# samuelskirvin/EIGENSOLVER

Measured on AMD Instinct MI355X. Metric: det(M) evals/sec + roots/sec, 4096x4096 (k,omega) grid, higher is better.
Workload: dtype f64

## Files before the change

### eigensolver_amd/csrc/es_shoot.hip

```cpp
#include <vector>
#include <cstdio>
#include <cstdlib>
#include <cmath>
#include <type_traits>

#include "es_shoot_shared.hpp"

namespace {
using namespace es_shoot_shared;

struct GridOpts {
  int skip;
  const int* cols;
  int part;
  int main_span;
};

constexpr long ES_TILE_GRID_X = 1L << 22;
__device__ __forceinline__ long es_tile_index() { return (long)blockIdx.y * ES_TILE_GRID_X + blockIdx.x; }
inline dim3 es_tile_grid(long tiles) {
  return tiles <= ES_TILE_GRID_X ? dim3((unsigned)tiles) : dim3((unsigned)ES_TILE_GRID_X, (unsigned)((tiles + ES_TILE_GRID_X - 1) / ES_TILE_GRID_X));
}

template <int FAM, int PTS, int MAXT, bool TRACK, int WPE = 0>
// ... 16 lines not shown
  constexpr int MAXT = 256;
#include "es_shoot_grid_body.hpp"
}

__device__ __forceinline__ bool column_dead(const ShootDev& P, double W) {
  const double m = 4.0 * 2.220446049250313e-16 * fabs(W);
  bool c = false;
  for (int t = 0; t < P.n_bands; ++t) {
    const bool some = (W - m > P.band[t][0]) && (W + m < P.band[t][3]);
    const bool notall = (W + m <= P.band[t][1]) || (W - m >= P.band[t][2]);
    c = c || (some && notall);
  }
  return c;
}

__global__ __launch_bounds__(1024) void column_classify_kernel(ShootDev P, const double* __restrict__ Wv, int nw,
                                                               int* __restrict__ cols, uint8_t* __restrict__ dead) {
  __shared__ int wave_cnt[16];
  __shared__ int base;
  const int tid = threadIdx.x, lane = tid & 63, wid = tid >> 6;
  if (tid == 0) base = 0;
  __syncthreads();
  for (int j0 = 0; j0 < nw; j0 += 1024) {
    const int j = j0 + tid;
    const bool in = j < nw;
    const bool dd = in && column_dead(P, Wv[j]);
    if (in) dead[j] = dd ? 1 : 0;
    const bool live = in && !dd;
    const uint64_t m = __ballot(live);
    if (lane == 0) wave_cnt[wid] = __popcll(m);
    __syncthreads();
    int off = base;
    for (int v = 0; v < wid; ++v) off += wave_cnt[v];
    const uint64_t lower = (lane == 0) ? 0ull : (~0ull >> (64 - lane));
    if (live) cols[1 + off + __popcll(m & lower)] = j;
    __syncthreads();
    if (tid == 0) { int t = 0; for (int v = 0; v < 16; ++v) t += wave_cnt[v]; base += t; }
    __syncthreads();
  }
  if (tid == 0) cols[0] = base;
}

__global__ __launch_bounds__(256) void fill_dead_columns_kernel(ShootDev P, const double* __restrict__ kv, int nk,
                                                                const double* __restrict__ wv, int nw,
                                                                const uint8_t* __restrict__ dead,
                                                                double* __restrict__ Dout, double* __restrict__ relout,
                                                                uint8_t* __restrict__ stout) {
  const long cells = (long)nk * nw;
  for (long c = (long)blockIdx.x * blockDim.x + threadIdx.x; c < cells; c += (long)gridDim.x * blockDim.x) {
    const long row = c / nw;
    const int j = (int)(c - row * nw);
    if (!dead[j]) continue;
    const double k = kv[row];
    const double w = k * wv[j];
    const double k2 = k * k;
    const double Oe = (P.family == FAM_CYL0 || P.family == FAM_CYLT) ? w : (w - k * P.U_e);
    const double Oe2 = Oe * Oe;
    const double m_e = ((k2 * P.vAe2 - Oe2) * (k2 * P.ce2 - Oe2)) / (P.Se * (k2 * P.cTe2 - Oe2));
    const double cst = (P.family == FAM_CYL0 || P.family == FAM_CYLT)
                           ? -1.0 / (P.rho_e * (k2 * P.vAe2 - w * w))
                           : P.rho_e * P.Se * (k2 * P.cTe2 - Oe2) / (Oe * (k2 * P.ce2 - Oe2));
    uint8_t st = ES_PT_CONTINUUM;
    if (m_e < 0.0) st = ES_PT_LEAKY;
    else if (!(m_e > 0.0) || !isfinite(m_e) || !isfinite(cst)) st = ES_PT_NONFINITE;
    Dout[c] = NAN;
    if (relout) relout[c] = NAN;
    stout[c] = st;
  }
}

template <int FAM>
__global__ __launch_bounds__(256) void shoot_points_kernel(ShootDev P, const double* __restrict__ kv,
                                                           const double* __restrict__ wv, const int* __restrict__ d_n,
                                                           int n_max, double* __restrict__ Dout,
                                                           double* __restrict__ relout, uint8_t* __restrict__ stout) {
  ES_POINT_LDS(FAM);
  const int n = es_count(d_n, n_max);
  if ((long)blockIdx.x * 256 >= (long)n) return;
  const int i = blockIdx.x * blockDim.x + threadIdx.x;
  const bool in = i < n;
  const double k = in ? kv[i] : 1.0;
  const double w = in ? wv[i] : 1.0;
  double D, rel; uint8_t st;
  shoot_point<FAM>(P, k, w, w, D, rel, st, es_point_lds);
  if (in) {
    Dout[i] = D;
    stout[i] = st;
    if (relout) relout[i] = rel;
  }
}

__global__ __launch_bounds__(256) void bracket_flag_kernel(const double* __restrict__ D,
                                                           const uint8_t* __restrict__ st, int nw, long cells,
                                                           uint64_t* __restrict__ masks,
                                                           int* __restrict__ block_counts) {
  __shared__ int wave_cnt[4];
  const long c = (long)blockIdx.x * 256 + threadIdx.x;
  const int lane = threadIdx.x & 63;
  double d0 = 0.0; int ok0 = 0;
  if (c < cells) { d0 = D[c]; ok0 = (st[c] == ES_PT_OK); }
  double d1 = __shfl_down(d0, 1);
  int ok1 = __shfl_down(ok0, 1);
  if (lane == 63) {
    if (c + 1 < cells) { d1 = D[c + 1]; ok1 = (st[c + 1] == ES_PT_OK); } else { d1 = 0.0; ok1 = 0; }
  }
  bool flag = false;
  if (c < cells) {
    const long row = c / nw;
    const int j = (int)(c - row * nw);
    flag = (j < nw - 1) && ok0 && ok1 && (d0 * d1 < 0.0);
  }
  const uint64_t m = __ballot(flag);
  if (lane == 0) {
    masks[c >> 6] = m;
    wave_cnt[threadIdx.x >> 6] = __popcll(m);
  }
  __syncthreads();
  if (threadIdx.x == 0) block_counts[blockIdx.x] = wave_cnt[0] + wave_cnt[1] + wave_cnt[2] + wave_cnt[3];
}

__global__ __launch_bounds__(256) void bracket_emit_kernel(const double* __restrict__ kv,
                                                           const double* __restrict__ wv, int nw, int w_mode,
                                                           long cells, const double* __restrict__ D,
                                                           const uint64_t* __restrict__ masks,
                                                           const int* __restrict__ block_off, es_root_table tab,
                                                           double* __restrict__ d_lo_sign, double* __restrict__ d_hi_sign) {
  const long c = (long)blockIdx.x * 256 + threadIdx.x;
  if (c >= cells) return;
  const uint64_t m = masks[c >> 6];
  if (!((m >> (c & 63)) & 1ull)) return;
  const int pos = es_cell_rank(masks, block_off, c);
  if (pos >= tab.capacity) return;
  const long row = c / nw;
  const int j = (int)(c - row * nw);
  const double k = kv[row];
  tab.d_k[pos] = k;
  tab.d_row[pos] = (int32_t)row;
  tab.d_w_lo[pos] = pick_w(wv, w_mode, k, (int)row, nw, j);
  tab.d_w_hi[pos] = pick_w(wv, w_mode, k, (int)row, nw, j + 1);
  d_lo_sign[pos] = D[c];
  d_hi_sign[pos] = D[c + 1];
}

constexpr int kRefineSections = 17;
constexpr int kSharedMin = 0;

constexpr int REFINE_WAVES = 4;

template <int FAM, int LANES, int CHR = 0, bool SECTIONS_ONLY = false, bool ONE = false,
          int WPE = ((FAM == FAM_CYLT || !ONE) ? 2 : 3)>
__global__ __launch_bounds__(64 * REFINE_WAVES) __attribute__((amdgpu_waves_per_eu(WPE, WPE)))
void refine_kernel(ShootDev P, es_root_table tab, double* d_lo, double* d_hi, const int* __restrict__ d_n, int n_max,
                   int n_rounds, int n_polish, double tol_percent) {
  const int n = es_count(d_n, n_max);
  if ((int)(blockIdx.x * REFINE_WAVES * (64 / LANES)) >= n) return;
  constexpr int GROUPS = 64 / LANES;
  constexpr int WTBL = GROUPS * (2 * (CHR > 0 ? CHR : 1) + 1) * FamTraits<FAM>::NE;
  __shared__ double es_point_lds[CHR > 0 ? REFINE_WAVES * WTBL : FamTraits<FAM>::NB * (2 * es_shoot_shared::CH + 1)];
  const int lane = threadIdx.x & 63;
  const int g = lane / LANES, j = lane % LANES;
  const int i = (blockIdx.x * REFINE_WAVES + ((int)threadIdx.x >> 6)) * GROUPS + g;
  const bool in = i < n;
  const double k = in ? tab.d_k[i] : 1.0;
  double lo = in ? tab.d_w_lo[i] : 1.0;
  double hi = in ? tab.d_w_hi[i] : 2.0;
  double flo = in ? d_lo[i] : 1.0;
  double fhi = in ? d_hi[i] : -1.0;
  const double frac = (double)(j + 1) / (double)(LANES + 1);
  double D = 0.0, rel = 0.0; uint8_t st = 0;
  double root = lo;
  const int n_final = (n_polish > 0) ? n_polish : (n_polish == 0 ? 1 : 0);
  const int n_it = ONE ? 1 : n_rounds + n_final;
  for (int it = 0; it < n_it; ++it) {
    const bool section = ONE ? true : it < n_rounds;
    double x;
    if (section) {
      x = lo + (hi - lo) * frac;
    } else if (n_polish > 0) {
      x = lo - flo * (hi - lo) / (fhi - flo);
      if (!(x > lo && x < hi)) x = (x == x) ? ((fabs(flo) <= fabs(fhi)) ? lo : hi) : lo + (hi - lo) * 0.5;
    } else {
      x = lo + (hi - lo) * 0.5;
    }
    if (CHR > 0) shoot_point_wavegroup<FAM, (CHR > 0 ? CHR : 1), GROUPS>(P, k, x, D, rel, st, es_point_lds + ((int)threadIdx.x >> 6) * WTBL);
    else if (SECTIONS_ONLY) shoot_point<FAM, false>(P, k, x, x, D, rel, st, es_point_lds);
    else shoot_point<FAM>(P, k, x, x, D, rel, st, es_point_lds);
    if (section) {
      const bool diff = (D * flo < 0.0);
      const unsigned long long bal = __ballot(diff);
      const unsigned long long bits = (LANES == 64) ? bal : ((bal >> (LANES * g)) & ((1ull << (LANES & 63)) - 1ull));
      const int first = bits ? (__ffsll((long long)bits) - 1) : LANES;
      const int src_hi = g * LANES + (first < LANES ? first : LANES - 1);
      const int src_lo = g * LANES + (first > 0 ? first - 1 : 0);
      const double x_hi = __shfl(x, src_hi), d_hi_new = __shfl(D, src_hi);
      const double x_lo = __shfl(x, src_lo), d_lo_new = __shfl(D, src_lo);
      if (first < LANES) { hi = x_hi; fhi = d_hi_new; }
      if (first > 0) { lo = x_lo; flo = (d_lo_new == d_lo_new) ? d_lo_new : flo; }
    } else {
      root = x;
      if (n_polish > 0) {
        if (D * flo < 0.0) { hi = x; fhi = D; } else if (D == D) { lo = x; flo = D; }
      }
    }
  }
  if (in && j == 0) {
    tab.d_w_lo[i] = lo;
    tab.d_w_hi[i] = hi;
    if (n_polish < 0) {
      d_lo[i] = flo;
      d_hi[i] = fhi;
    } else {
      tab.d_w[i] = root;
      tab.d_resid[i] = rel;
      tab.d_flag[i] = (st == ES_PT_OK && rel < tol_percent) ? 1 : 0;
    }
  }
}

template <int FAM, bool ONE = false, int WPE = ((FAM == FAM_CYLT || !ONE) ? 2 : 3)>
__global__ __launch_bounds__(64 * REFINE_WAVES) __attribute__((amdgpu_waves_per_eu(WPE, WPE)))
void refine_polish_kernel(ShootDev P, es_root_table tab, double* d_lo, double* d_hi, const int* __restrict__ d_n,
                          int n_max, int n_polish, double tol_percent) {
  ES_POINT_LDS(FAM);
  const int n = es_count(d_n, n_max);
  if ((int)(blockIdx.x * (64 * REFINE_WAVES)) >= n) return;
  const int i = blockIdx.x * (64 * REFINE_WAVES) + (int)threadIdx.x;
  const bool in = i < n;
  const double k = in ? tab.d_k[i] : 1.0;
  double lo = in ? tab.d_w_lo[i] : 1.0;
  double hi = in ? tab.d_w_hi[i] : 2.0;
  double flo = in ? d_lo[i] : 1.0;
  double fhi = in ? d_hi[i] : -1.0;
  double D = 0.0, rel = 0.0; uint8_t st = 0;
  double root = lo;
  const int n_it = ONE ? 1 : n_polish;
  for (int it = 0; it < n_it; ++it) {
    double x = lo - flo * (hi - lo) / (fhi - flo);
    if (!(x > lo && x < hi)) x = (x == x) ? ((fabs(flo) <= fabs(fhi)) ? lo : hi) : lo + (hi - lo) * 0.5;
    shoot_point<FAM>(P, k, x, x, D, rel, st, es_point_lds);
    root = x;
    if (D * flo < 0.0) { hi = x; fhi = D; } else if (D == D) { lo = x; flo = D; }
  }
  if (in) {
    tab.d_w_lo[i] = lo;
    tab.d_w_hi[i] = hi;
    if (ONE && n_polish == 0) {
      d_lo[i] = flo;
      d_hi[i] = fhi;
    } else {
      tab.d_w[i] = root;
      tab.d_resid[i] = rel;
      tab.d_flag[i] = (st == ES_PT_OK && rel < tol_percent) ? 1 : 0;
    }
  }
}

constexpr int kHybridSections = 1;
constexpr int kHybridSteps = 8;
constexpr double kHybridEps = 1e-12;

struct HybridState {
  double* lo; double* hi; double* flo; double* fhi; double* xprev;
  int* info;
};
constexpr int HYB_ACTIVE = 0, HYB_KEPT = 1, HYB_FAILED = 2;

template <int FAM, int WPE = (FAM == FAM_CYL0 ? 3 : 2)>
__global__ __launch_bounds__(64 * REFINE_WAVES) __attribute__((amdgpu_waves_per_eu(WPE, WPE)))
void refine_superlinear_kernel(ShootDev P, es_root_table tab, const double* d_lo, const double* d_hi, HybridState S,
                               const int* __restrict__ d_n, int n_max, int step, double tol_percent,
                               unsigned long long* stats) {
  ES_POINT_LDS(FAM);
  const int n = es_count(d_n, n_max);
  if ((int)(blockIdx.x * (64 * REFINE_WAVES)) >= n) return;
  const int i = blockIdx.x * (64 * REFINE_WAVES) + (int)threadIdx.x;
  const bool in = i < n;
  const bool first = step == 0;
  const int info = (in && !first) ? S.info[i] : 0;
  const bool active = in && ((info >> 2) == HYB_ACTIVE);
  if (!__syncthreads_or(active ? 1 : 0)) return;
  const double k = in ? tab.d_k[i] : 1.0;
  double lo, hi, flo, fhi, xprev;
  if (first) {
    lo = in ? tab.d_w_lo[i] : 1.0;
    hi = in ? tab.d_w_hi[i] : 2.0;
    flo = in ? d_lo[i] : 1.0;
    fhi = in ? d_hi[i] : -1.0;
    xprev = NAN;
  } else {
    lo = active ? S.lo[i] : 1.0;
    hi = active ? S.hi[i] : 2.0;
    flo = active ? S.flo[i] : 1.0;
    fhi = active ? S.fhi[i] : -1.0;
    xprev = active ? S.xprev[i] : NAN;
  }
  int side = info & 3, status = info >> 2;
  double D = 0.0, rel = 0.0; uint8_t st = 0;
  double x = lo - flo * (hi - lo) / (fhi - flo);
  if (!(x > lo && x < hi)) x = lo + (hi - lo) * 0.5;
  shoot_point<FAM>(P, k, x, x, D, rel, st, es_point_lds);
  if (active) {
    if (D == D) {
      if (D * flo < 0.0) { hi = x; fhi = D; if (side == 1) flo *= 0.5; side = 1; }
      else { lo = x; flo = D; if (side == 2) fhi *= 0.5; side = 2; }
      const double ax = fabs(x);
      if (D == 0.0 || fabs(x - xprev) <= kHybridEps * ax || (hi - lo) <= kHybridEps * ax)
        status = (st == ES_PT_OK && rel < tol_percent) ? HYB_KEPT : HYB_FAILED;
    } else {
      status = HYB_FAILED;
    }
    if (status == HYB_KEPT) {
      tab.d_w_lo[i] = lo;
      tab.d_w_hi[i] = hi;
      tab.d_w[i] = x;
      tab.d_resid[i] = rel;
      tab.d_flag[i] = 1;
    } else if (status == HYB_ACTIVE) {
      S.lo[i] = lo; S.hi[i] = hi; S.flo[i] = flo; S.fhi[i] = fhi; S.xprev[i] = x;
    }
    S.info[i] = side | (status << 2);
  }
  const int n_eval = __popcll(__ballot(active)), n_kept = __popcll(__ballot(active && status == HYB_KEPT));
  if ((threadIdx.x & 63) == 0) {
    if (first && n_eval) atomicAdd(stats + 0, (unsigned long long)n_eval);
    if (n_kept) atomicAdd(stats + 1, (unsigned long long)n_kept);
    if (n_eval) atomicAdd(stats + 3, (unsigned long long)n_eval);
  }
}

__global__ __launch_bounds__(256) void hybrid_flag_kernel(const int* __restrict__ info, const int* __restrict__ d_n,
                                                          int n_max, uint64_t* __restrict__ masks,
                                                          int* __restrict__ block_counts, unsigned long long* stats) {
  __shared__ int wave_cnt[4];
  const int n = es_count(d_n, n_max);
  const int i = blockIdx.x * 256 + (int)threadIdx.x;
  const bool flag = i < n && (info[i] >> 2) != HYB_KEPT;
  const uint64_t m = __ballot(flag);
  if ((threadIdx.x & 63) == 0) {
    masks[i >> 6] = m;
    wave_cnt[threadIdx.x >> 6] = __popcll(m);
  }
  __syncthreads();
  if (threadIdx.x == 0) {
    const int c = wave_cnt[0] + wave_cnt[1] + wave_cnt[2] + wave_cnt[3];
    block_counts[blockIdx.x] = c;
    if (c) atomicAdd(stats + 2, (unsigned long long)c);
  }
}

__global__ __launch_bounds__(256) void hybrid_gather_kernel(es_root_table tab, es_root_table ftab, int* __restrict__ idx,
                                                            const uint64_t* __restrict__ masks,
                                                            const int* __restrict__ block_off,
                                                            const int* __restrict__ d_n, int n_max) {
  const int n = es_count(d_n, n_max);
  const int i = blockIdx.x * 256 + (int)threadIdx.x;
  if (i >= n) return;
  if (!((masks[i >> 6] >> (i & 63)) & 1ull)) return;
  const int pos = es_cell_rank(masks, block_off, (long)i);
  if (pos >= ftab.capacity) return;
  ftab.d_k[pos] = tab.d_k[i];
  ftab.d_w_lo[pos] = tab.d_w_lo[i];
  ftab.d_w_hi[pos] = tab.d_w_hi[i];
  ftab.d_w[pos] = tab.d_w[i];
  ftab.d_resid[pos] = tab.d_resid[i];
  ftab.d_row[pos] = tab.d_row[i];
  idx[pos] = i;
}

__global__ __launch_bounds__(256) void hybrid_scatter_kernel(es_root_table ftab, es_root_table tab,
// ... 514 lines not shown
GridShape pick_shape(int nw, bool track) {
  GridShape best{4, 2};
  double best_cost = 1e300;
  for (int pts : {4, 3, 2, 1}) {
    if (ShapeTable<FAM>::wpe[pts] == 0) continue;
    const int T = shape_threads(nw, pts);
    const long span = (long)T * pts;
    const long padded = (nw + span - 1) / span * span;
    static const double wave_count_cost[5] = {0.0, 1.83, 1.39, 1.17, 1.0};
    const double c = (double)padded * ShapeTable<FAM>::cost[pts] * wave_count_cost[T / 64];
    if (c < best_cost) { best_cost = c; best = GridShape{pts, ShapeTable<FAM>::wpe[pts]}; }
  }
  if (track && fam_has_bands<FAM>()) best.wpe = 2;
  if (const char* ev = getenv("ES_GRID_SHAPE")) {
    int p = 0, w = 0;
    if (sscanf(ev, "%d,%d", &p, &w) == 2 && p >= 1 && p <= 4 && w >= 2 && w <= 4) best = GridShape{p, w};
  }
  return best;
}

template <int FAM, int PTS, int WPE, bool TRACK>
constexpr bool shape_built() {
  if (PTS == 3 && ShapeTable<FAM>::wpe[3] == 0) return false;
#if defined(ES_ALL_GRID_SHAPES)
  return true;
#else
  if (TRACK && fam_has_bands<FAM>()) return WPE == 2;
  if (FAM == FAM_CYL0 && PTS == 4 && WPE == 2) return true;
  return ShapeTable<FAM>::wpe[PTS] == WPE;
#endif
}

template <int FAM>
bool rows2_shape(int nw, bool track) {
  if (!fam_has_bands<FAM>() || track || nw > 512) return false;
  const char* r2 = getenv("ES_GRID_ROWS2");
  return !(r2 && r2[0] == '0') && !getenv("ES_GRID_SHAPE");
}

template <int FAM>
int launch_grid(es_context* ctx, const es_problem* prob, const double* d_k, int nk, const double* d_w, int nw,
                int w_mode, double* d_D, double* d_rel, uint8_t* d_status, int flags = 0) {
  GridOpts opts;
  opts.skip = (flags & ES_EVAL_SKIP_CONTINUUM) ? 1 : 0;
  opts.cols = nullptr;
  opts.part = 0;
  opts.main_span = 0;
  if (opts.skip && w_mode == ES_W_PHASE_SPEED && fam_has_bands<FAM>() && prob->dev.use_bands) {
    if ((size_t)nw + 1 > ctx->cols_cap) {
      ES_HIP_CHECK(ctx, hipStreamSynchronize(ctx->stream));
      if (ctx->d_cols) ES_HIP_CHECK(ctx, hipFree(ctx->d_cols));
      if (ctx->d_coldead) ES_HIP_CHECK(ctx, hipFree(ctx->d_coldead));
      ctx->d_cols = nullptr; ctx->d_coldead = nullptr; ctx->cols_cap = 0;
      ES_HIP_CHECK(ctx, hipMalloc(&ctx->d_cols, ((size_t)nw + 1) * sizeof(int)));
      ES_HIP_CHECK(ctx, hipMalloc(&ctx->d_coldead, (size_t)nw));
      ctx->cols_cap = (size_t)nw + 1;
    }
    hipLaunchKernelGGL(column_classify_kernel, dim3(1), dim3(1024), 0, ctx->stream, prob->dev, d_w, nw, ctx->d_cols,
                       ctx->d_coldead);
    ES_HIP_CHECK(ctx, hipGetLastError());
    const long cells = (long)nk * nw;
    const int fb = (int)((cells + 255) / 256 < 8192 ? (cells + 255) / 256 : 8192);
    hipLaunchKernelGGL(fill_dead_columns_kernel, dim3(fb), dim3(256), 0, ctx->stream, prob->dev, d_k, nk, d_w, nw,
                       ctx->d_coldead, d_D, d_rel, d_status);
    ES_HIP_CHECK(ctx, hipGetLastError());
    opts.cols = ctx->d_cols;
  }
  const bool track = !(fam_has_bands<FAM>() && prob->dev.use_bands);
  GridShape shape = pick_shape<FAM>(nw, track);
  const int T = shape_threads(nw, shape.pts);
  const long tiles = (long)nk * ((nw + (long)T * shape.pts - 1) / ((long)T * shape.pts));
  const dim3 grid = es_tile_grid(tiles);
  bool launched = false;
  es_timer_begin(ctx);
  if constexpr (fam_has_bands<FAM>()) {
    if (rows2_shape<FAM>(nw, track) && !opts.cols && nk >= 2) {
      const int pts2 = (nw + 127) / 128;
      const dim3 grid2 = es_tile_grid(((long)nk + 1) / 2);
#define ES_R2(P_)                                                                                                   \
      if (pts2 == P_) hipLaunchKernelGGL((shoot_grid_kernel_r2<FAM, P_, false, 3>), grid2, dim3(256), 0, ctx->stream, \
                                         prob->dev, d_k, nk, d_w, nw, w_mode, d_D, d_rel, d_status, opts);
      ES_R2(1) ES_R2(2) ES_R2(3) ES_R2(4)
#undef ES_R2
      launched = true;
    }
  }
  auto one = [&](auto pts_c, auto wpe_c, auto track_c) {
    constexpr int PTS = decltype(pts_c)::value, WPE = decltype(wpe_c)::value;
    constexpr bool TRACK = decltype(track_c)::value;
    if constexpr (shape_built<FAM, PTS, WPE, TRACK>() && (TRACK || fam_has_bands<FAM>())) {
      if (launched || shape.pts != PTS || shape.wpe != WPE || track != TRACK) return;
      launched = true;
      if constexpr (FAM == FAM_CYL0 && PTS == 4 && !TRACK) {
        if (opts.cols && T > 64) {
          opts.part = 1;
          hipLaunchKernelGGL((shoot_grid_kernel<FAM, PTS, 256, TRACK, WPE>), grid, dim3(T), 0, ctx->stream,
                             prob->dev, d_k, nk, d_w, nw, w_mode, d_D, d_rel, d_status, opts);
          opts.part = 2;
          opts.main_span = 4 * T;
          const long tiles2 = (long)nk * (T / 64);
          hipLaunchKernelGGL((shoot_grid_kernel<FAM, 4, 64, false, 2>), es_tile_grid(tiles2),
                             dim3(64), 0, ctx->stream, prob->dev, d_k, nk, d_w, nw, w_mode, d_D, d_rel, d_status, opts);
          return;
        }
      }
      hipLaunchKernelGGL((shoot_grid_kernel<FAM, PTS, 256, TRACK, WPE>), grid, dim3(T), 0, ctx->stream, prob->dev,
                         d_k, nk, d_w, nw, w_mode, d_D, d_rel, d_status, opts);
    }
  };
  using std::integral_constant;
#define ES_SHAPE(P_, W_)                                                                                            \
  one(integral_constant<int, P_>{}, integral_constant<int, W_>{}, integral_constant<bool, false>{});                \
  one(integral_constant<int, P_>{}, integral_constant<int, W_>{}, integral_constant<bool, true>{});
  ES_SHAPE(4, 2) ES_SHAPE(4, 3) ES_SHAPE(4, 4) ES_SHAPE(3, 2) ES_SHAPE(3, 3) ES_SHAPE(2, 2) ES_SHAPE(2, 3) ES_SHAPE(2, 4) ES_SHAPE(1, 2) ES_SHAPE(1, 3) ES_SHAPE(1, 4)
#undef ES_SHAPE
  es_timer_end(ctx);
  if (!launched) {
    ctx->last_error = "grid launch shape not built (ES_GRID_SHAPE names a shape outside this build)";
    return ES_ERR_UNSUPPORTED;
  }
  ES_HIP_CHECK(ctx, hipGetLastError());
  return ES_SUCCESS;
}

inline int es_bound(long n_max) { return (int)(n_max < INT32_MAX ? n_max : INT32_MAX); }
inline dim3 es_blocks(long n_max) { return dim3((unsigned)((n_max + 255) / 256)); }

template <int FAM>
int launch_points(es_context* ctx, const es_problem* prob, const double* d_k, const double* d_w, const int* d_n, long n_max,
                  double* d_D, double* d_rel, uint8_t* d_status) {
  hipLaunchKernelGGL((shoot_points_kernel<FAM>), es_blocks(n_max), dim3(256), 0, ctx->stream, prob->dev, d_k, d_w, d_n,
                     es_bound(n_max), d_D, d_rel, d_status);
  ES_HIP_CHECK(ctx, hipGetLastError());
  return ES_SUCCESS;
}

int dispatch_points(es_context* ctx, const es_problem* prob, const double* d_k, const double* d_w, const int* d_n, long n_max,
                    double* d_D, double* d_rel, uint8_t* d_status) {
#define CALL_PTS(F) launch_points<F>(ctx, prob, d_k, d_w, d_n, n_max, d_D, d_rel, d_status)
  ES_DISPATCH_FAMILY(prob->dev.family, CALL_PTS)
#undef CALL_PTS
}

template <int FAM>
int launch_refine_steps(es_context* ctx, const es_problem* prob, const es_root_table& tab, double* d_lo, double* d_hi,
                        const int* d_n, int n_max, int n_hint, int sections, int rounds, int np, bool polish, double tol) {
  constexpr int CHR = (FAM == FAM_CYL0) ? 32 : 0;
  int shared_min = kSharedMin;
  if (const char* ev = getenv("ES_REFINE_SHARED_MIN")) shared_min = atoi(ev);
  const bool shared_entries = CHR > 0 && np < 0 && n_hint >= shared_min && !getenv("ES_REFINE_PRIVATE_ENTRIES");
  auto blocks = [&](int per_wg) { return dim3((n_max + per_wg - 1) / per_wg); };
  constexpr bool ONE_ROUND_FAM = (FAM == FAM_CYLT || FAM == FAM_CYL0);
  const bool one_round = ONE_ROUND_FAM && !getenv("ES_REFINE_ROUNDS_IN_KERNEL");
#define ES_REFINE(LANES_, CHR_, SO_, PER_WG_)                                                                           \
  if (SO_ && one_round) {                                                                                               \
    if constexpr (ONE_ROUND_FAM && SO_) {                                                                               \
      for (int r_ = 0; r_ < rounds; ++r_)                                                                               \
        hipLaunchKernelGGL((refine_kernel<FAM, LANES_, CHR_, true, true>), blocks(PER_WG_), dim3(64 * REFINE_WAVES), 0, \
                           ctx->stream, prob->dev, tab, d_lo, d_hi, d_n, n_max, 1, np, tol);                            \
    }                                                                                                                   \
  } else                                                                                                                \
    hipLaunchKernelGGL((refine_kernel<FAM, LANES_, CHR_, SO_, false>), blocks(PER_WG_), dim3(64 * REFINE_WAVES), 0,     \
                       ctx->stream, prob->dev, tab, d_lo, d_hi, d_n, n_max, rounds, np, tol)
  if (sections == 17 && shared_entries) ES_REFINE(16, CHR, true, 4 * REFINE_WAVES);
  else if (np < 0) {
    if (sections == 17) ES_REFINE(16, 0, true, 4 * REFINE_WAVES);
    else if (sections == 9) ES_REFINE(8, 0, true, 8 * REFINE_WAVES);
    else ES_REFINE(4, 0, true, 16 * REFINE_WAVES);
  } else {
    if (sections == 17) ES_REFINE(16, 0, false, 4 * REFINE_WAVES);
    else if (sections == 9) ES_REFINE(8, 0, false, 8 * REFINE_WAVES);
    else ES_REFINE(4, 0, false, 16 * REFINE_WAVES);
  }
#undef ES_REFINE
  ES_HIP_CHECK(ctx, hipGetLastError());
  if (np < 0 && polish) {
    if (one_round) {
      if constexpr (ONE_ROUND_FAM) {
        for (int p_ = 0; p_ < ES_REFINE_POLISH; ++p_)
          hipLaunchKernelGGL((refine_polish_kernel<FAM, true>), blocks(64 * REFINE_WAVES), dim3(64 * REFINE_WAVES), 0, ctx->stream,
                             prob->dev, tab, d_lo, d_hi, d_n, n_max, p_ == ES_REFINE_POLISH - 1 ? 1 : 0, tol);
      }
    } else
      hipLaunchKernelGGL((refine_polish_kernel<FAM, false>), blocks(64 * REFINE_WAVES), dim3(64 * REFINE_WAVES), 0, ctx->stream,
                         prob->dev, tab, d_lo, d_hi, d_n, n_max, ES_REFINE_POLISH, tol);
    ES_HIP_CHECK(ctx, hipGetLastError());
  }
  return ES_SUCCESS;
}

int refine_sections() {
  int sections = kRefineSections;
  if (const char* ev = getenv("ES_REFINE_SECTIONS")) {
    const int v = atoi(ev);
    if (v == 5 || v == 9 || v == 17) sections = v;
  }
  return sections;
}

int check_refine_rule(es_context* ctx) {
  if (ctx->refine_rule == ES_REFINE_HYBRID && refine_sections() != kRefineSections) {
    ctx->last_error = "ES_REFINE_HYBRID is defined for 17-section only (ES_REFINE_SECTIONS is set to another rule)";
    return ES_ERR_UNSUPPORTED;
  }
  return ES_SUCCESS;
}

template <int FAM>
int launch_refine_hybrid(es_context* ctx, const es_problem* prob, const es_root_table& tab, const int* d_n, int n_max,
                         int n_hint, int rounds, double tol) {
  if (n_max <= 0) return ES_SUCCESS;
  auto align = [](size_t b) { return (b + 255) & ~(size_t)255; };
  const size_t cap = (size_t)n_max;
  const size_t bd = align(cap * sizeof(double)), bi = align(cap * sizeof(int)), bf = align(cap);
  const int nblk = (n_max + 255) / 256;
  const size_t bm = align((size_t)nblk * 4 * sizeof(uint64_t)), bc = align((size_t)(nblk + 1) * sizeof(int));
  int rc = es_ensure_hybrid_scratch(ctx, 10 * bd + 3 * bi + bf + bm + bc + 256);
  if (rc) return rc;
  char* b = (char*)ctx->d_hybrid;
  auto take = [&](size_t bytes) { char* p = b; b += bytes; return p; };
  HybridState S;
  S.lo = (double*)take(bd); S.hi = (double*)take(bd); S.flo = (double*)take(bd); S.fhi = (double*)take(bd);
  S.xprev = (double*)take(bd);
  S.info = (int*)take(bi);
  es_root_table ftab;
  ftab.d_k = (double*)take(bd); ftab.d_w = (double*)take(bd); ftab.d_w_lo = (double*)take(bd);
  ftab.d_w_hi = (double*)take(bd); ftab.d_resid = (double*)take(bd);
  ftab.d_row = (int32_t*)take(bi); ftab.d_flag = (uint8_t*)take(bf);
  ftab.capacity = n_max;
  int* idx = (int*)take(bi);
  uint64_t* masks = (uint64_t*)take(bm);
  int* counts = (int*)take(bc);
  int* d_nf = (int*)take(256);
  rc = launch_refine_steps<FAM>(ctx, prob, tab, tab.d_w, tab.d_resid, d_n, n_max, n_hint, kRefineSections, kHybridSections,
                                -1, false, tol);
  if (rc) return rc;
  const dim3 wg(64 * REFINE_WAVES), grid((n_max + 64 * REFINE_WAVES - 1) / (64 * REFINE_WAVES));
  for (int s_ = 0; s_ < kHybridSteps; ++s_)
    hipLaunchKernelGGL((refine_superlinear_kernel<FAM>), grid, wg, 0, ctx->stream, prob->dev, tab, tab.d_w, tab.d_resid, S,
                       d_n, n_max, s_, tol, ctx->d_refine_stats);
  ES_HIP_CHECK(ctx, hipGetLastError());
  hipLaunchKernelGGL(hybrid_flag_kernel, dim3(nblk), dim3(256), 0, ctx->stream, S.info, d_n, n_max, masks, counts,
                     ctx->d_refine_stats);
  ES_HIP_CHECK(ctx, hipGetLastError());
  rc = es_scan_counts_async(ctx, counts, nblk, d_nf);
  if (rc) return rc;
  hipLaunchKernelGGL(hybrid_gather_kernel, dim3(nblk), dim3(256), 0, ctx->stream, tab, ftab, idx, masks, counts, d_n, n_max);
  ES_HIP_CHECK(ctx, hipGetLastError());
  rc = launch_refine_steps<FAM>(ctx, prob, ftab, ftab.d_w, ftab.d_resid, d_nf, n_max, n_hint, kRefineSections,
                                rounds - kHybridSections, -1, true, tol);
  if (rc) return rc;
  hipLaunchKernelGGL(hybrid_scatter_kernel, dim3(nblk), dim3(256), 0, ctx->stream, ftab, tab, idx, d_nf, n_max);
  ES_HIP_CHECK(ctx, hipGetLastError());
  return ES_SUCCESS;
}

template <int FAM>
int launch_refine(es_context* ctx, const es_problem* prob, const es_root_table& tab, double* d_lo, double* d_hi,
                  const int* d_n, int n_max, int n_hint, int n_bisect, double tol) {
  const int sections = refine_sections();
  int rounds = 0;
  for (double span = 1.0, need = ldexp(1.0, n_bisect < 1000 ? n_bisect : 1000); span < need; span *= (double)sections) ++rounds;
  if (ctx->refine_rule == ES_REFINE_HYBRID) {
    const int rc = check_refine_rule(ctx);
    if (rc) return rc;
    if (rounds > kHybridSections) return launch_refine_hybrid<FAM>(ctx, prob, tab, d_n, n_max, n_hint, rounds, tol);
  }
  const int np = (ES_REFINE_POLISH > 0 && rounds > 0) ? -1 : ES_REFINE_POLISH;
  return launch_refine_steps<FAM>(ctx, prob, tab, d_lo, d_hi, d_n, n_max, n_hint, sections, rounds, np, true, tol);
}

int dispatch_refine(es_context* ctx, const es_problem* prob, const es_root_table& tab, const int* d_n, int n_max, int n_hint,
                    int n_bisect, double tol) {
#define CALL_REFINE(F) launch_refine<F>(ctx, prob, tab, tab.d_w, tab.d_resid, d_n, n_max, n_hint, n_bisect, tol)
  ES_DISPATCH_FAMILY(prob->dev.family, CALL_REFINE)
#undef CALL_REFINE
}

}

extern "C" int es_problem_create(es_context* ctx, const es_shoot_desc* d, const es_profiles* pr, es_problem** out) {
  if (!ctx) return ES_ERR_INVALID_ARG;
  ES_REQUIRE(ctx, d && pr && out, "null pointer");
  *out = nullptr;
  ES_REQUIRE(ctx, d->n_nodes >= 2 && d->n_nodes <= (1 << 24), "n_nodes out of range");
  ES_REQUIRE(ctx, d->geometry >= 0 && d->geometry <= 3, "geometry");
  ES_REQUIRE(ctx, d->x_boundary == -1.0 || d->x_boundary == 1.0, "x_boundary must be -1 or +1");
  const int N = d->n_nodes, npts = 2 * N - 1;
  int nb = 0;
  switch (d->geometry) {
    case ES_GEOM_CYLINDER: nb = FamTraits<FAM_CYL0>::NB; break;
    case ES_GEOM_CYLINDER_TWIST: nb = FamTraits<FAM_CYLT>::NB; break;
    case ES_GEOM_SLAB_DENSITY: nb = FamTraits<FAM_SLABD>::NB; break;
    default: nb = FamTraits<FAM_SLABF>::NB; break;
  }
  std::vector<double> base((size_t)nb * npts);
  auto B = [&](int f, int i) -> double& { return base[(size_t)f * npts + i]; };
  if (d->geometry == ES_GEOM_CYLINDER || d->geometry == ES_GEOM_CYLINDER_TWIST) {
    ES_REQUIRE(ctx, pr->r && pr->rho && pr->c2 && pr->Bz, "cylinder profiles r, rho, c2, Bz required");
    ES_REQUIRE(ctx, d->axis_bc >= 0 && d->axis_bc <= 2, "axis_bc");
    ES_REQUIRE(ctx, d->c1_power == 1 || d->c1_power == 2, "c1_power");
    ES_REQUIRE(ctx, d->m >= 0 && d->m_ext >= 0 && d->m_ext <= 64, "m");
    for (int i = 0; i < npts; ++i) {
      const double r = pr->r[i], rho = pr->rho[i], c2 = pr->c2[i], Bz = pr->Bz[i];
      const double Bphi = pr->Bphi ? pr->Bphi[i] : 0.0;
      const double vz = pr->vz ? pr->vz[i] : 0.0;
      const double vphi = pr->vphi ? pr->vphi[i] : 0.0;
      const double sr = sqrt(rho);
      const double bA = Bz / sr;
      const double vA = (Bz + Bphi) / sr;
      const double S = c2 + vA * vA;
      const double q = c2 / S;
      if (d->geometry == ES_GEOM_CYLINDER) {
        ES_REQUIRE(ctx, Bphi == 0.0 && vphi == 0.0, "ES_GEOM_CYLINDER needs Bphi = vphi = 0 (use CYLINDER_TWIST)");
        B(C0_VZ, i) = vz;
        B(C0_BA, i) = bA;
        B(C0_Q, i) = q;
        B(C0_A1, i) = rho / r;
        B(C0_B1, i) = r / (rho * S);
        B(C0_E1, i) = 1.0 / (r * rho);
        B(C0_E2, i) = r / rho;
      } else {
        const double dm = (double)d->m, dm2 = dm * dm;
        const double invr = 1.0 / r, invr2 = invr * invr;
        const double bphr = Bphi / r, vphr = vphi / r;
        const double Bphi_n = bphr * r, vphi_n = vphr * r;
        B(CT_MB, i) = dm * bphr;
// ... 597 lines not shown
```

### eigensolver_amd/csrc/es_shoot_shared.hpp

```cpp
#pragma once
#include "es_common.hpp"
#include "es_shoot_device.hpp"

struct es_problem {
  ShootDev dev;
  double* d_base = nullptr;
  es_shoot_desc desc;
};

namespace es_shoot_shared {

constexpr int ES_REFINE_POLISH = 2;
#if defined(ES_STAGE_FAR_NODE_ALWAYS)
#define ES_FAR_NODE(c_, n_) 1
#else
#define ES_FAR_NODE(c_, n_) (((c_) == (n_) - 1) ? 1 : 0)
#endif
constexpr int CH = 128;

template <int FAM>
__device__ __forceinline__ void load_base(const ShootDev& P, int pt, double* b) {
#pragma unroll
  for (int f = 0; f < FamTraits<FAM>::NB; ++f) b[f] = P.base[(size_t)f * P.npts + pt];
}
// ... 71 lines not shown
        Coef Bm, B1;
        ES_ENTRY(2 * j + 1, e)
        ES_ENTRY(2 * j, e2)
        coefficients2<FAM, TRACK, C1P>(e, e2, P, s, w, Bm, B1, trk);
        adjoint_step<FAM>(zp, zq, B0, Bm, B1, h, h2, h6, h3);
        B0 = B1;
        --j;
      }
      if (j >= 1) {
        double e1[NE], em2[NE];
        Coef Cm, C1, Cm2, C2;
        ES_ENTRY(2 * j + 1, e)
        ES_ENTRY(2 * j, e1)
        ES_ENTRY(2 * j - 1, em2)
        ES_ENTRY(2 * j - 2, e2)
        coefficients4<FAM, TRACK>(e, e1, em2, e2, P, s, w, Cm, C1, Cm2, C2, trk);
        for (; j >= 3; j -= 2) {
          Coef Nm, N1, Nm2, N2;
          ES_ENTRY(2 * j - 3, e)
          ES_ENTRY(2 * j - 4, e1)
          ES_ENTRY(2 * j - 5, em2)
          ES_ENTRY(2 * j - 6, e2)
          coefficients4<FAM, TRACK>(e, e1, em2, e2, P, s, w, Nm, N1, Nm2, N2, trk);
          adjoint_step<FAM>(zp, zq, B0, Cm, C1, h, h2, h6, h3);
          adjoint_step<FAM>(zp, zq, C1, Cm2, C2, h, h2, h6, h3);
          B0 = C2;
          Cm = Nm; C1 = N1; Cm2 = Nm2; C2 = N2;
        }
        adjoint_step<FAM>(zp, zq, B0, Cm, C1, h, h2, h6, h3);
        adjoint_step<FAM>(zp, zq, C1, Cm2, C2, h, h2, h6, h3);
        B0 = C2;
      }
    } else {
      Coef Cm, C1;
      ES_ENTRY(2 * j + 1, e)
      ES_ENTRY(2 * j, e2)
      coefficients2<FAM, TRACK, C1P>(e, e2, P, s, w, Cm, C1, trk);
      for (; j >= 1; --j) {
        Coef Nm, N1;
        ES_ENTRY(2 * j - 1, e)
        ES_ENTRY(2 * j - 2, e2)
        coefficients2<FAM, TRACK, C1P>(e, e2, P, s, w, Nm, N1, trk);
        adjoint_step<FAM>(zp, zq, B0, Cm, C1, h, h2, h6, h3);
        B0 = C1;
        Cm = Nm; C1 = N1;
      }
      adjoint_step<FAM>(zp, zq, B0, Cm, C1, h, h2, h6, h3);
      B0 = C1;
    }
#undef ES_ENTRY
    adjoint_rescale<FAM>(zp, zq, nsteps - c0 - nst, nsteps - c0);
  }
  const Mismatch M = boundary_algebra<FAM>(P, s, w, X, zp, zq, e2);
  finish_point(P, M, X, TRACK ? trk.crossed() : (BANDS ? band_crossed(P, k, w) : false), D, rel, st);
}

template <int FAM, bool TRACK, int CHR, int NG>
__device__ __forceinline__ void shoot_point_wavegroup_impl(const ShootDev& P, double k, double w, double& D, double& rel,
                                                           uint8_t& st, double* __restrict__ tbl) {
  constexpr int NE = FamTraits<FAM>::NE;
  constexpr int NB = FamTraits<FAM>::NB;
  constexpr int NODES = 2 * CHR + 1;
  constexpr int GL = 64 / NG;
  const int lane = threadIdx.x & 63;
  const int grp = lane / GL;
  const KScal s = make_kscal(P, k);
  const int nsteps = P.n_nodes - 1;
  const double h = P.h, h2 = 0.5 * P.h, h6 = P.h / 6.0, h3 = P.h / 3.0;
  SignTrack trk;
  double e[NE], e2[NE];
  const ExteriorLite X = exterior_lite(P, k, w, w);
  Coef B0;
  double zp = 0.0, zq = 0.0;
  const double* mine = tbl + (size_t)grp * NODES * NE;
  double kgs[NG];
#pragma unroll
  for (int g2 = 0; g2 < NG; ++g2) kgs[g2] = __shfl(k, g2 * GL);
  const int nchunks = (nsteps + CHR - 1) / CHR;
  for (int c = nchunks - 1; c >= 0; --c) {
    const int c0 = c * CHR;
    const int nst = (nsteps - c0 < CHR) ? (nsteps - c0) : CHR;
    const int nn = 2 * nst + ES_FAR_NODE(c, nchunks);
    __builtin_amdgcn_wave_barrier();
    for (int idx = lane; idx < NG * nn; idx += 64) {
      const int g2 = idx / nn, i = idx - g2 * nn;
      double kg = kgs[0];
#pragma unroll
      for (int q = 1; q < NG; ++q) kg = (g2 == q) ? kgs[q] : kg;
      const KScal sg = make_kscal(P, kg);
      double b[NB], eg[NE];
#pragma unroll
      for (int f = 0; f < NB; ++f) b[f] = P.base[(size_t)f * P.npts + 2 * c0 + i];
      make_entry<FAM, fam_scaled<FAM>()>(b, sg, eg);
#pragma unroll
      for (int f = 0; f < NE; ++f) tbl[((size_t)g2 * NODES + i) * NE + f] = eg[f];
    }
    __builtin_amdgcn_wave_barrier();
    if (c == nchunks - 1) {
#pragma unroll
      for (int f = 0; f < NE; ++f) e[f] = mine[2 * nst * NE + f];
      coefficients<FAM, TRACK>(e, P, s, w, B0, trk);
      adjoint_start(P, B0, zp, zq);
    }
    int j = nst - 1;
    if (!fam_rcp4<FAM>() || !(j & 1)) {
      for (; j >= 0 && (!fam_rcp4<FAM>() || !(j & 1)); --j) {
        Coef Bm, B1;
#pragma unroll
        for (int f = 0; f < NE; ++f) { e[f] = mine[(2 * j + 1) * NE + f]; e2[f] = mine[2 * j * NE + f]; }
        coefficients2<FAM, TRACK>(e, e2, P, s, w, Bm, B1, trk);
        adjoint_step<FAM>(zp, zq, B0, Bm, B1, h, h2, h6, h3);
        B0 = B1;
      }
    }
    if (fam_rcp4<FAM>() && j >= 1) {
      double e1[NE], em2[NE];
      Coef Cm, C1, Cm2, C2;
#pragma unroll
      for (int f = 0; f < NE; ++f) {
        e[f] = mine[(2 * j + 1) * NE + f]; e1[f] = mine[2 * j * NE + f];
        em2[f] = mine[(2 * j - 1) * NE + f]; e2[f] = mine[(2 * j - 2) * NE + f];
      }
      coefficients4<FAM, TRACK>(e, e1, em2, e2, P, s, w, Cm, C1, Cm2, C2, trk);
      for (; j >= 3; j -= 2) {
        Coef Nm, N1, Nm2, N2;
#pragma unroll
        for (int f = 0; f < NE; ++f) {
          e[f] = mine[(2 * j - 3) * NE + f]; e1[f] = mine[(2 * j - 4) * NE + f];
          em2[f] = mine[(2 * j - 5) * NE + f]; e2[f] = mine[(2 * j - 6) * NE + f];
        }
        coefficients4<FAM, TRACK>(e, e1, em2, e2, P, s, w, Nm, N1, Nm2, N2, trk);
        adjoint_step<FAM>(zp, zq, B0, Cm, C1, h, h2, h6, h3);
        adjoint_step<FAM>(zp, zq, C1, Cm2, C2, h, h2, h6, h3);
        B0 = C2;
        Cm = Nm; C1 = N1; Cm2 = Nm2; C2 = N2;
      }
      adjoint_step<FAM>(zp, zq, B0, Cm, C1, h, h2, h6, h3);
      adjoint_step<FAM>(zp, zq, C1, Cm2, C2, h, h2, h6, h3);
      B0 = C2;
    }
    adjoint_rescale<FAM>(zp, zq, nsteps - c0 - nst, nsteps - c0);
  }
  const Mismatch M = boundary_algebra<FAM>(P, s, w, X, zp, zq, e2);
  finish_point(P, M, X, TRACK ? trk.crossed() : band_crossed(P, k, w), D, rel, st);
}

template <int FAM, int CHR, int NG>
__device__ __forceinline__ void shoot_point_wavegroup(const ShootDev& P, double k, double w, double& D, double& rel,
                                                      uint8_t& st, double* __restrict__ tbl) {
  if (fam_has_bands<FAM>() && P.use_bands) shoot_point_wavegroup_impl<FAM, !fam_has_bands<FAM>(), CHR, NG>(P, k, w, D, rel, st, tbl);
  else shoot_point_wavegroup_impl<FAM, true, CHR, NG>(P, k, w, D, rel, st, tbl);
}

template <int FAM, bool STATUS = true>
__device__ __forceinline__ void shoot_point(const ShootDev& P, double k, double w, double w_cst, double& D,
                                            double& rel, uint8_t& st, double* __restrict__ sb) {
  if (FAM == FAM_CYLT) {
    if (!STATUS) {
      if (P.c1_power == 2) shoot_point_impl<FAM, false, false, 2>(P, k, w, w_cst, D, rel, st, sb);
      else shoot_point_impl<FAM, false, false, 1>(P, k, w, w_cst, D, rel, st, sb);
    } else {
      if (P.c1_power == 2) shoot_point_impl<FAM, true, false, 2>(P, k, w, w_cst, D, rel, st, sb);
      else shoot_point_impl<FAM, true, false, 1>(P, k, w, w_cst, D, rel, st, sb);
    }
  } else if (!STATUS) {
    shoot_point_impl<FAM, false, false>(P, k, w, w_cst, D, rel, st, sb);
  } else if (fam_has_bands<FAM>() && P.use_bands) shoot_point_impl<FAM, !fam_has_bands<FAM>()>(P, k, w, w_cst, D, rel, st, sb);
  else shoot_point_impl<FAM, true>(P, k, w, w_cst, D, rel, st, sb);
}

#define ES_POINT_LDS(FAM) __shared__ double es_point_lds[FamTraits<FAM>::NB * (2 * es_shoot_shared::CH + 1)]

}
```

Baseline: 852.0 million.

## Add wave-table refine kernel with padded, 16-byte aligned LDS node entries

Adds a new refine kernel for the shared-entries path (CYL0, 17 sections). Each wave builds node coefficient entries for all its groups into an LDS table whose per-field rows are padded to an even stride and 16-byte aligned. The adjoint sweep then reads node pairs as double2 vector loads and interleaves coefficient computation with adjoint steps in a software-pipelined loop. The aim is fewer, wider LDS reads and better overlap. It becomes the default for that path; the old wavegroup path stays behind an env var, and the refine body is moved into a shared include file.

```diff
diff --git a/eigensolver_amd/csrc/es_shoot.hip b/eigensolver_amd/csrc/es_shoot.hip
--- a/eigensolver_amd/csrc/es_shoot.hip
+++ b/eigensolver_amd/csrc/es_shoot.hip
@@ -192,69 +192,22 @@
 __global__ __launch_bounds__(64 * REFINE_WAVES) __attribute__((amdgpu_waves_per_eu(WPE, WPE)))
 void refine_kernel(ShootDev P, es_root_table tab, double* d_lo, double* d_hi, const int* __restrict__ d_n, int n_max,
                    int n_rounds, int n_polish, double tol_percent) {
-  const int n = es_count(d_n, n_max);
-  if ((int)(blockIdx.x * REFINE_WAVES * (64 / LANES)) >= n) return;
-  constexpr int GROUPS = 64 / LANES;
-  constexpr int WTBL = GROUPS * (2 * (CHR > 0 ? CHR : 1) + 1) * FamTraits<FAM>::NE;
-  __shared__ double es_point_lds[CHR > 0 ? REFINE_WAVES * WTBL : FamTraits<FAM>::NB * (2 * es_shoot_shared::CH + 1)];
-  const int lane = threadIdx.x & 63;
-  const int g = lane / LANES, j = lane % LANES;
-  const int i = (blockIdx.x * REFINE_WAVES + ((int)threadIdx.x >> 6)) * GROUPS + g;
-  const bool in = i < n;
-  const double k = in ? tab.d_k[i] : 1.0;
-  double lo = in ? tab.d_w_lo[i] : 1.0;
-  double hi = in ? tab.d_w_hi[i] : 2.0;
-  double flo = in ? d_lo[i] : 1.0;
-  double fhi = in ? d_hi[i] : -1.0;
-  const double frac = (double)(j + 1) / (double)(LANES + 1);
-  double D = 0.0, rel = 0.0; uint8_t st = 0;
-  double root = lo;
-  const int n_final = (n_polish > 0) ? n_polish : (n_polish == 0 ? 1 : 0);
-  const int n_it = ONE ? 1 : n_rounds + n_final;
-  for (int it = 0; it < n_it; ++it) {
-    const bool section = ONE ? true : it < n_rounds;
-    double x;
-    if (section) {
-      x = lo + (hi - lo) * frac;
-    } else if (n_polish > 0) {
-      x = lo - flo * (hi - lo) / (fhi - flo);
-      if (!(x > lo && x < hi)) x = (x == x) ? ((fabs(flo) <= fabs(fhi)) ? lo : hi) : lo + (hi - lo) * 0.5;
-    } else {
-      x = lo + (hi - lo) * 0.5;
-    }
-    if (CHR > 0) shoot_point_wavegroup<FAM, (CHR > 0 ? CHR : 1), GROUPS>(P, k, x, D, rel, st, es_point_lds + ((int)threadIdx.x >> 6) * WTBL);
-    else if (SECTIONS_ONLY) shoot_point<FAM, false>(P, k, x, x, D, rel, st, es_point_lds);
-    else shoot_point<FAM>(P, k, x, x, D, rel, st, es_point_lds);
-    if (section) {
-      const bool diff = (D * flo < 0.0);
-      const unsigned long long bal = __ballot(diff);
-      const unsigned long long bits = (LANES == 64) ? bal : ((bal >> (LANES * g)) & ((1ull << (LANES & 63)) - 1ull));
-      const int first = bits ? (__ffsll((long long)bits) - 1) : LANES;
-      const int src_hi = g * LANES + (first < LANES ? first : LANES - 1);
-      const int src_lo = g * LANES + (first > 0 ? first - 1 : 0);
-      const double x_hi = __shfl(x, src_hi), d_hi_new = __shfl(D, src_hi);
-      const double x_lo = __shfl(x, src_lo), d_lo_new = __shfl(D, src_lo);
-      if (first < LANES) { hi = x_hi; fhi = d_hi_new; }
-      if (first > 0) { lo = x_lo; flo = (d_lo_new == d_lo_new) ? d_lo_new : flo; }
-    } else {
-      root = x;
-      if (n_polish > 0) {
-        if (D * flo < 0.0) { hi = x; fhi = D; } else if (D == D) { lo = x; flo = D; }
-      }
-    }
-  }
-  if (in && j == 0) {
-    tab.d_w_lo[i] = lo;
-    tab.d_w_hi[i] = hi;
-    if (n_polish < 0) {
-      d_lo[i] = flo;
-      d_hi[i] = fhi;
-    } else {
-      tab.d_w[i] = root;
-      tab.d_resid[i] = rel;
-      tab.d_flag[i] = (st == ES_PT_OK && rel < tol_percent) ? 1 : 0;
-    }
-  }
+  constexpr bool WAVETABLE = false;
+#define ES_REFINE_LDS_ALIGN
+#include "es_shoot_refine_body.hpp"
+#undef ES_REFINE_LDS_ALIGN
+}
+
+template <int FAM, int LANES, int CHR, bool SECTIONS_ONLY = true, bool ONE = false,
+          int WPE = ((FAM == FAM_CYLT || !ONE) ? 2 : 3)>
+__global__ __launch_bounds__(64 * REFINE_WAVES) __attribute__((amdgpu_waves_per_eu(WPE, WPE)))
+void refine_wavetable_kernel(ShootDev P, es_root_table tab, double* d_lo, double* d_hi, const int* __restrict__ d_n, int n_max,
+                             int n_rounds, int n_polish, double tol_percent) {
+  static_assert(CHR > 0, "wave-shared node entries only");
+  constexpr bool WAVETABLE = true;
+#define ES_REFINE_LDS_ALIGN __attribute__((aligned(16)))
+#include "es_shoot_refine_body.hpp"
+#undef ES_REFINE_LDS_ALIGN
 }
 
 template <int FAM, bool ONE = false, int WPE = ((FAM == FAM_CYLT || !ONE) ? 2 : 3)>
@@ -1075,18 +1028,21 @@
   auto blocks = [&](int per_wg) { return dim3((n_max + per_wg - 1) / per_wg); };
   constexpr bool ONE_ROUND_FAM = (FAM == FAM_CYLT || FAM == FAM_CYL0);
   const bool one_round = ONE_ROUND_FAM && !getenv("ES_REFINE_ROUNDS_IN_KERNEL");
-#define ES_REFINE(LANES_, CHR_, SO_, PER_WG_)                                                                           \
+#define ES_REFINE_K(KERNEL_, LANES_, CHR_, SO_, PER_WG_)                                                                \
   if (SO_ && one_round) {                                                                                               \
     if constexpr (ONE_ROUND_FAM && SO_) {                                                                               \
       for (int r_ = 0; r_ < rounds; ++r_)                                                                               \
-        hipLaunchKernelGGL((refine_kernel<FAM, LANES_, CHR_, true, true>), blocks(PER_WG_), dim3(64 * REFINE_WAVES), 0, \
+        hipLaunchKernelGGL((KERNEL_<FAM, LANES_, CHR_, true, true>), blocks(PER_WG_), dim3(64 * REFINE_WAVES), 0,       \
                            ctx->stream, prob->dev, tab, d_lo, d_hi, d_n, n_max, 1, np, tol);                            \
     }                                                                                                                   \
   } else                                                                                                                \
-    hipLaunchKernelGGL((refine_kernel<FAM, LANES_, CHR_, SO_, false>), blocks(PER_WG_), dim3(64 * REFINE_WAVES), 0,     \
+    hipLaunchKernelGGL((KERNEL_<FAM, LANES_, CHR_, SO_, false>), blocks(PER_WG_), dim3(64 * REFINE_WAVES), 0,           \
                        ctx->stream, prob->dev, tab, d_lo, d_hi, d_n, n_max, rounds, np, tol)
-  if (sections == 17 && shared_entries) ES_REFINE(16, CHR, true, 4 * REFINE_WAVES);
-  else if (np < 0) {
+#define ES_REFINE(LANES_, CHR_, SO_, PER_WG_) ES_REFINE_K(refine_kernel, LANES_, CHR_, SO_, PER_WG_)
+  if (sections == 17 && shared_entries) {
+    if (getenv("ES_REFINE_WAVEGROUP_ENTRIES")) { ES_REFINE(16, CHR, true, 4 * REFINE_WAVES); }
+    else if constexpr (CHR > 0) { ES_REFINE_K(refine_wavetable_kernel, 16, CHR, true, 4 * REFINE_WAVES); }
+  } else if (np < 0) {
     if (sections == 17) ES_REFINE(16, 0, true, 4 * REFINE_WAVES);
     else if (sections == 9) ES_REFINE(8, 0, true, 8 * REFINE_WAVES);
     else ES_REFINE(4, 0, true, 16 * REFINE_WAVES);
@@ -1096,6 +1052,7 @@
     else ES_REFINE(4, 0, false, 16 * REFINE_WAVES);
   }
 #undef ES_REFINE
+#undef ES_REFINE_K
   ES_HIP_CHECK(ctx, hipGetLastError());
   if (np < 0 && polish) {
     if (one_round) {
diff --git a/eigensolver_amd/csrc/es_shoot_refine_body.hpp b/eigensolver_amd/csrc/es_shoot_refine_body.hpp
--- /dev/null
+++ b/eigensolver_amd/csrc/es_shoot_refine_body.hpp
@@ -0,0 +1,67 @@
+  const int n = es_count(d_n, n_max);
+  if ((int)(blockIdx.x * REFINE_WAVES * (64 / LANES)) >= n) return;
+  constexpr int GROUPS = 64 / LANES;
+  constexpr int WTBL = WAVETABLE ? wavetable_doubles<FAM, (CHR > 0 ? CHR : 1), GROUPS>()
+                                 : GROUPS * (2 * (CHR > 0 ? CHR : 1) + 1) * FamTraits<FAM>::NE;
+  __shared__ ES_REFINE_LDS_ALIGN double es_point_lds[CHR > 0 ? REFINE_WAVES * WTBL : FamTraits<FAM>::NB * (2 * es_shoot_shared::CH + 1)];
+  const int lane = threadIdx.x & 63;
+  const int g = lane / LANES, j = lane % LANES;
+  const int i = (blockIdx.x * REFINE_WAVES + ((int)threadIdx.x >> 6)) * GROUPS + g;
+  const bool in = i < n;
+  const double k = in ? tab.d_k[i] : 1.0;
+  double lo = in ? tab.d_w_lo[i] : 1.0;
+  double hi = in ? tab.d_w_hi[i] : 2.0;
+  double flo = in ? d_lo[i] : 1.0;
+  double fhi = in ? d_hi[i] : -1.0;
+  const double frac = (double)(j + 1) / (double)(LANES + 1);
+  double D = 0.0, rel = 0.0; uint8_t st = 0;
+  double root = lo;
+  const int n_final = (n_polish > 0) ? n_polish : (n_polish == 0 ? 1 : 0);
+  const int n_it = ONE ? 1 : n_rounds + n_final;
+  for (int it = 0; it < n_it; ++it) {
+    const bool section = ONE ? true : it < n_rounds;
+    double x;
+    if (section) {
+      x = lo + (hi - lo) * frac;
+    } else if (n_polish > 0) {
+      x = lo - flo * (hi - lo) / (fhi - flo);
+      if (!(x > lo && x < hi)) x = (x == x) ? ((fabs(flo) <= fabs(fhi)) ? lo : hi) : lo + (hi - lo) * 0.5;
+    } else {
+      x = lo + (hi - lo) * 0.5;
+    }
+    if (CHR > 0) {
+      if constexpr (WAVETABLE) shoot_point_wavetable<FAM, (CHR > 0 ? CHR : 1), GROUPS>(P, k, x, D, rel, st, es_point_lds + ((int)threadIdx.x >> 6) * WTBL);
+      else shoot_point_wavegroup<FAM, (CHR > 0 ? CHR : 1), GROUPS>(P, k, x, D, rel, st, es_point_lds + ((int)threadIdx.x >> 6) * WTBL);
+    }
+    else if (SECTIONS_ONLY) shoot_point<FAM, false>(P, k, x, x, D, rel, st, es_point_lds);
+    else shoot_point<FAM>(P, k, x, x, D, rel, st, es_point_lds);
+    if (section) {
+      const bool diff = (D * flo < 0.0);
+      const unsigned long long bal = __ballot(diff);
+      const unsigned long long bits = (LANES == 64) ? bal : ((bal >> (LANES * g)) & ((1ull << (LANES & 63)) - 1ull));
+      const int first = bits ? (__ffsll((long long)bits) - 1) : LANES;
+      const int src_hi = g * LANES + (first < LANES ? first : LANES - 1);
+      const int src_lo = g * LANES + (first > 0 ? first - 1 : 0);
+      const double x_hi = __shfl(x, src_hi), d_hi_new = __shfl(D, src_hi);
+      const double x_lo = __shfl(x, src_lo), d_lo_new = __shfl(D, src_lo);
+      if (first < LANES) { hi = x_hi; fhi = d_hi_new; }
+      if (first > 0) { lo = x_lo; flo = (d_lo_new == d_lo_new) ? d_lo_new : flo; }
+    } else {
+      root = x;
+      if (n_polish > 0) {
+        if (D * flo < 0.0) { hi = x; fhi = D; } else if (D == D) { lo = x; flo = D; }
+      }
+    }
+  }
+  if (in && j == 0) {
+    tab.d_w_lo[i] = lo;
+    tab.d_w_hi[i] = hi;
+    if (n_polish < 0) {
+      d_lo[i] = flo;
+      d_hi[i] = fhi;
+    } else {
+      tab.d_w[i] = root;
+      tab.d_resid[i] = rel;
+      tab.d_flag[i] = (st == ES_PT_OK && rel < tol_percent) ? 1 : 0;
+    }
+  }
diff --git a/eigensolver_amd/csrc/es_shoot_shared.hpp b/eigensolver_amd/csrc/es_shoot_shared.hpp
--- a/eigensolver_amd/csrc/es_shoot_shared.hpp
+++ b/eigensolver_amd/csrc/es_shoot_shared.hpp
@@ -247,6 +247,129 @@
   else shoot_point_wavegroup_impl<FAM, true, CHR, NG>(P, k, w, D, rel, st, tbl);
 }
 
+template <int CHR> constexpr int wavetable_lstride() { return 2 * CHR + 2; }
+template <int FAM, int CHR, int NG> constexpr int wavetable_doubles() { return NG * FamTraits<FAM>::NE * wavetable_lstride<CHR>(); }
+
+template <int FAM, bool TRACK, int CHR, int NG>
+__device__ __forceinline__ void shoot_point_wavetable_impl(const ShootDev& P, double k, double w, double& D, double& rel,
+                                                           uint8_t& st, double* __restrict__ tbl) {
+  typedef double es_d2 __attribute__((ext_vector_type(2)));
+  constexpr int NE = FamTraits<FAM>::NE;
+  constexpr int NB = FamTraits<FAM>::NB;
+  constexpr int LS = wavetable_lstride<CHR>();
+  constexpr int GL = 64 / NG;
+  static_assert(2 * CHR <= 64, "the nodes of a chunk are one build pass of 64 lanes (plus the far node)");
+  const int lane = threadIdx.x & 63;
+  const int grp = lane / GL;
+  const KScal s = make_kscal(P, k);
+  const int nsteps = P.n_nodes - 1;
+  const double h = P.h, h2 = 0.5 * P.h, h6 = P.h / 6.0, h3 = P.h / 3.0;
+  SignTrack trk;
+  double e[NE], e1[NE], em2[NE], e2[NE];
+  const ExteriorLite X = exterior_lite(P, k, w, w);
+  Coef B0;
+  double zp = 0.0, zq = 0.0;
+  const double* mine = tbl + grp * (NE * LS);
+  double kgs[NG];
+#pragma unroll
+  for (int g2 = 0; g2 < NG; ++g2)
+    kgs[g2] = __hiloint2double(__builtin_amdgcn_readlane(__double2hiint(k), g2 * GL),
+                               __builtin_amdgcn_readlane(__double2loint(k), g2 * GL));
+#define ES_WG_LOAD4(J)                                                                         \
+  _Pragma("unroll") for (int f = 0; f < NE; ++f) {                                             \
+    const es_d2 u_ = *reinterpret_cast<const es_d2*>(mine + f * LS + 2 * (J));                 \
+    const es_d2 l_ = *reinterpret_cast<const es_d2*>(mine + f * LS + 2 * (J) - 2);             \
+    e[f] = u_.y; e1[f] = u_.x; em2[f] = l_.y; e2[f] = l_.x;                                    \
+  }
+  const int nchunks = (nsteps + CHR - 1) / CHR;
+  for (int c = nchunks - 1; c >= 0; --c) {
+    const int c0 = c * CHR;
+    const int nst = (nsteps - c0 < CHR) ? (nsteps - c0) : CHR;
+    const int nn = 2 * nst + ES_FAR_NODE(c, nchunks);
+    __builtin_amdgcn_wave_barrier();
+    KScal sg[NG];
+#pragma unroll
+    for (int g2 = 0; g2 < NG; ++g2) {
+      double kg = kgs[g2];
+      asm volatile("" : "+s"(kg));
+      sg[g2] = make_kscal(P, kg);
+    }
+    for (int i = lane; i < nn; i += 64) {
+      double b[NB];
+      load_base<FAM>(P, 2 * c0 + i, b);
+#pragma unroll
+      for (int g2 = 0; g2 < NG; ++g2) {
+        double eg[NE];
+        make_entry<FAM, fam_scaled<FAM>()>(b, sg[g2], eg);
+#pragma unroll
+        for (int f = 0; f < NE; ++f) tbl[(g2 * NE + f) * LS + i] = eg[f];
+      }
+    }
+    __builtin_amdgcn_wave_barrier();
+    if (c == nchunks - 1) {
+#pragma unroll
+      for (int f = 0; f < NE; ++f) e[f] = mine[f * LS + 2 * nst];
+      coefficients<FAM, TRACK>(e, P, s, w, B0, trk);
+      adjoint_start(P, B0, zp, zq);
+    }
+    int j = nst - 1;
+    if (!fam_rcp4<FAM>() || !(j & 1)) {
+      for (; j >= 0 && (!fam_rcp4<FAM>() || !(j & 1)); --j) {
+        Coef Bm, B1;
+#pragma unroll
+        for (int f = 0; f < NE; ++f) {
+          const es_d2 u_ = *reinterpret_cast<const es_d2*>(mine + f * LS + 2 * j);
+          e[f] = u_.y; e2[f] = u_.x;
+        }
+        coefficients2<FAM, TRACK>(e, e2, P, s, w, Bm, B1, trk);
+        adjoint_step<FAM>(zp, zq, B0, Bm, B1, h, h2, h6, h3);
+        B0 = B1;
+      }
+    }
+    if (fam_rcp4<FAM>() && j >= 1) {
+      Coef Am, A1, Am2, A2, Bm, B1, Bm2, B2;
+      ES_WG_LOAD4(j)
+      coefficients4<FAM, TRACK>(e, e1, em2, e2, P, s, w, Am, A1, Am2, A2, trk);
+      for (; j >= 5; j -= 4) {
+        adjoint_step<FAM>(zp, zq, B0, Am, A1, h, h2, h6, h3);
+        ES_WG_LOAD4(j - 2)
+        coefficients4<FAM, TRACK>(e, e1, em2, e2, P, s, w, Bm, B1, Bm2, B2, trk);
+        adjoint_step<FAM>(zp, zq, A1, Am2, A2, h, h2, h6, h3);
+        __builtin_amdgcn_sched_barrier(0);
+        adjoint_step<FAM>(zp, zq, A2, Bm, B1, h, h2, h6, h3);
+        ES_WG_LOAD4(j - 4)
+        coefficients4<FAM, TRACK>(e, e1, em2, e2, P, s, w, Am, A1, Am2, A2, trk);
+        adjoint_step<FAM>(zp, zq, B1, Bm2, B2, h, h2, h6, h3);
+        B0 = B2;
+      }
+      if (j == 3) {
+        adjoint_step<FAM>(zp, zq, B0, Am, A1, h, h2, h6, h3);
+        ES_WG_LOAD4(1)
+        coefficients4<FAM, TRACK>(e, e1, em2, e2, P, s, w, Bm, B1, Bm2, B2, trk);
+        adjoint_step<FAM>(zp, zq, A1, Am2, A2, h, h2, h6, h3);
+        B0 = A2;
+        Am = Bm; A1 = B1; Am2 = Bm2; A2 = B2;
+      }
+      adjoint_step<FAM>(zp, zq, B0, Am, A1, h, h2, h6, h3);
+      adjoint_step<FAM>(zp, zq, A1, Am2, A2, h, h2, h6, h3);
+      B0 = A2;
+    }
+    adjoint_rescale<FAM>(zp, zq, nsteps - c0 - nst, nsteps - c0);
+  }
+#undef ES_WG_LOAD4
+#pragma unroll
+  for (int f = 0; f < NE; ++f) e2[f] = mine[f * LS];
+  const Mismatch M = boundary_algebra<FAM>(P, s, w, X, zp, zq, e2);
+  finish_point(P, M, X, TRACK ? trk.crossed() : band_crossed(P, k, w), D, rel, st);
+}
+
+template <int FAM, int CHR, int NG>
+__device__ __forceinline__ void shoot_point_wavetable(const ShootDev& P, double k, double w, double& D, double& rel,
+                                                      uint8_t& st, double* __restrict__ tbl) {
+  if (fam_has_bands<FAM>() && P.use_bands) shoot_point_wavetable_impl<FAM, !fam_has_bands<FAM>(), CHR, NG>(P, k, w, D, rel, st, tbl);
+  else shoot_point_wavetable_impl<FAM, true, CHR, NG>(P, k, w, D, rel, st, tbl);
+}
+
 template <int FAM, bool STATUS = true>
 __device__ __forceinline__ void shoot_point(const ShootDev& P, double k, double w, double w_cst, double& D,
                                             double& rel, uint8_t& st, double* __restrict__ sb) {
```

After: 857.2 million, median of 6. No clear change (+0.6%).
